# JeffOwOSun/ntm-tracker

Hardware: AMD Instinct MI355X
Metric: frames/sec (whole node) VGG16+NTM(128x20) seq_len=20 (higher is better)
Workload: dtype f32

## Files before the change

ntm-tracker_amd/csrc/conv_bf16p.hip:

```cpp
#include "conv_tiles.h"
#include "conv_stem.h"

#ifndef BF16P_ABL
#define BF16P_ABL 0
#endif

namespace {

typedef __bf16 pbf16x8 __attribute__((ext_vector_type(8)));
typedef __bf16 pbf16x4 __attribute__((ext_vector_type(4)));


struct Bf16pArgs {
    const __bf16* in; const __bf16* wq; const float* bias; void* out;
    int frames, H, W, Cin, Cout;
    int bxN, byN;
    int NQ, NS;
    int nCB;
    const float* stem_in = nullptr; const float* stem_w = nullptr; const float* stem_b = nullptr;
};

typedef int pv4i __attribute__((ext_vector_type(4)));
__device__ __forceinline__ void p_dma16(pv4i rs, unsigned lds_addr, int voff, int soff) {
    unsigned keep;
    asm volatile("s_mov_b32 %0, m0\n\ts_mov_b32 m0, %1\n\ts_nop 0\n\tbuffer_load_dwordx4 %2, %3, %4 offen lds\n\ts_mov_b32 m0, %0"
                 : "=&s"(keep) : "s"(lds_addr), "v"(voff), "s"(rs), "s"(soff) : "memory");
}
__device__ __forceinline__ pv4i p_rsrc(const void* base, unsigned bytes) {
    const unsigned long long p = (unsigned long long)base;
    return pv4i{(int)(unsigned)p, (int)(unsigned)(p >> 32), (int)bytes, 0x00020000};
}

__device__ __forceinline__ pbf16x8 p_as_bf16x8(const f32x4& v) {
    union { f32x4 f; pbf16x8 b; } u;
    u.f = v;
    return u.b;
}

typedef _Float16 ph16x8 __attribute__((ext_vector_type(8)));
typedef _Float16 ph16x4 __attribute__((ext_vector_type(4)));
typedef _Float16 ph16x2 __attribute__((ext_vector_type(2)));
__device__ __forceinline__ ph16x8 p_as_f16x8(const f32x4& v) {
    union { f32x4 f; ph16x8 h; } u;
    u.f = v;
    return u.h;
}
__device__ __forceinline__ void s3_split4(const f32x4& v, ph16x4& hi, ph16x4& lo) {
    const auto h01 = __builtin_amdgcn_cvt_pkrtz(v[0], v[1]), h23 = __builtin_amdgcn_cvt_pkrtz(v[2], v[3]);
    hi = ph16x4{(_Float16)h01[0], (_Float16)h01[1], (_Float16)h23[0], (_Float16)h23[1]};
#pragma unroll
    for (int e = 0; e < 4; ++e) lo[e] = (_Float16)(v[e] - (float)hi[e]);
}
constexpr float S3_MAX = 131008.f;

template <int PIECES>
__device__ __forceinline__ int p_sw(int idx) { return PIECES == 4 ? ((idx >> 2) & 3) : ((idx >> 3) & 1); }

template <int BN, int KC>
__global__ void bf16p_pack_kernel(const float* __restrict__ w, __bf16* __restrict__ wq, int Cin, int Cout) {
    constexpr int PIECES = KC / 8;
    const size_t total = (size_t)9 * Cin * Cout;
    const int NC = Cin / KC;
    for (size_t idx = (size_t)blockIdx.x * blockDim.x + threadIdx.x; idx < total; idx += (size_t)gridDim.x * blockDim.x) {
        const int e = idx & 7;
        size_t r = idx >> 3;
        const int slot = (int)(r % PIECES); r /= PIECES;
        const int n = (int)(r % BN); r /= BN;
        const int tap = (int)(r % 9); r /= 9;
        const int chunk = (int)(r % NC);
        const int cb = (int)(r / NC);
        const int piece = slot ^ p_sw<PIECES>(n);
        const int c = chunk * KC + piece * 8 + e;
        wq[idx] = (__bf16)w[((size_t)tap * Cin + c) * Cout + (size_t)cb * BN + n];
    }
}

__global__ void split3_absmax_kernel(const float* __restrict__ w, size_t n, unsigned* __restrict__ tail) {
    float m = 0.f;
    for (size_t i = (size_t)blockIdx.x * blockDim.x + threadIdx.x; i < n; i += (size_t)gridDim.x * blockDim.x) {
        const float v = fabsf(w[i]);
        if (v < 3.0e38f) m = fmaxf(m, v);
    }
#pragma unroll
    for (int o = 32; o > 0; o >>= 1) m = fmaxf(m, __shfl_xor(m, o));
    if ((threadIdx.x & 63) == 0) atomicMax(tail + 1, __float_as_uint(m));
}
__global__ void split3_scale_kernel(unsigned* __restrict__ tail) {
    const float m = __uint_as_float(tail[1]);
    int e = 0;
    if (m > 0.f) frexpf(m, &e);
    int k = 14 - e;
    k = k > 100 ? 100 : (k < -100 ? -100 : k);
    reinterpret_cast<float*>(tail)[0] = ldexpf(1.f, -k);
    reinterpret_cast<float*>(tail)[2] = ldexpf(1.f, k);
}
template <int BN>
__global__ void split3_pack_kernel(const float* __restrict__ w, _Float16* __restrict__ wq, int Cin, int Cout) {
    const size_t total = (size_t)18 * Cin * Cout;
    const float wscale = reinterpret_cast<const float*>(wq + total)[2];
    const int NC = Cin / 16;
    for (size_t idx = (size_t)blockIdx.x * blockDim.x + threadIdx.x; idx < total; idx += (size_t)gridDim.x * blockDim.x) {
        const int e = idx & 7;
        size_t r = idx >> 3;
        const int slot = (int)(r & 3); r >>= 2;
        const int n = (int)(r % BN); r /= BN;
        const int tap = (int)(r % 9); r /= 9;
        const int chunk = (int)(r % NC);
        const int cb = (int)(r / NC);
        const int piece = slot ^ p_sw<4>(n);
        const int c = chunk * 16 + (piece & 1) * 8 + e;
        const float v = w[((size_t)tap * Cin + c) * Cout + (size_t)cb * BN + n] * wscale;
        const _Float16 hi = (_Float16)v;
        wq[idx] = (piece & 2) ? (_Float16)(v - (float)hi) : hi;
    }
}

template <int BN, int TW, int TH, int NSUB, int KC, bool POOL, bool OUTF32, int NW = 8, bool X3 = false, bool INF32 = false, bool STEM = false>
__global__ __launch_bounds__(64 * NW) __attribute__((amdgpu_waves_per_eu(2, 2))) void conv3x3_relu_bf16p_kernel(Bf16pArgs a) {
    static_assert(!INF32 || (X3 && NW == 4), "fp32 input: split form on four waves (the eight-wave form has no registers for the staging)");
    static_assert(!STEM || (X3 && NW == 4 && !INF32 && (TW & (TW - 1)) == 0 && TW % 2 == 0), "fused stem: split form on four waves, sub-blocks");
    constexpr int PNT = 2 * NW;
    constexpr bool ROWS = (TW & (TW - 1)) != 0;
    static_assert(!X3 || KC == 32, "split form: 16 real channels = one 32-channel chunk");
    static_assert(!ROWS || (!POOL && NSUB == 1 && (TW - 1 + 32 * PNT - 1) / TW + 1 <= TH - 1 && NW == 8), "runs of rows: no row pairs; TH = the patch's image rows");
    static_assert(NW == 8 || (NW == 4 && BN == 64), "four-wave workgroups take 64 columns");
    constexpr int PW = ROWS ? 32 : TW + 2, PH = TH + 2, SPX = PW * PH, NPX = NSUB * SPX;
    static_assert(!ROWS || TW + 2 <= 32, "runs of rows: the patch row pitch is 32");
    constexpr int PIXB = KC * 2, PIECES = KC / 8, PPP = 1024 / PIXB;
    constexpr int NPA = (NPX + PPP - 1) / PPP;
    constexpr int ABYTES = STEM ? NPX * PIXB : NPA * 1024;
    constexpr int STAPS = KC == 16 ? 9 : 3, SPC = 9 / STAPS;
    constexpr int SBYTES = STAPS * BN * PIXB, NPB = SBYTES / 1024;
    constexpr int NPAW = (NPA + NW - 1) / NW;
    constexpr int TM = BN == 128 ? 4 : 2;
    constexpr int TPS = (TW * TH) / 32;
    constexpr int K16 = KC / 16;
    static_assert(ROWS || NSUB * TW * TH == 32 * PNT, "512 (256) output pixels per workgroup");
    constexpr int TRB = POOL ? 0 : NW * TM * 32 * 144;
    constexpr int LDSB = (2 * ABYTES + 2 * SBYTES) > TRB ? (2 * ABYTES + 2 * SBYTES) : TRB;
    constexpr int FPW = TW + 4, FPN = STEM ? NSUB * (TH + 4) * FPW * 3 : 4;
    constexpr int STEMB = STEM ? (FPN + 4 * 27 * 16 + 64) * 4 : 0;
    static_assert(LDSB + STEMB + 1024 <= ((NW == 8 || (STEM && NSUB > 1)) ? 160 : 80) * 1024, "LDS");
    __shared__ __attribute__((aligned(16))) float s_fp[FPN];
    __shared__ __attribute__((aligned(16))) float s_w1[STEM ? 4 * 27 * 16 : 4];
    __shared__ __attribute__((aligned(16))) float s_b1[STEM ? 64 : 4];
    __shared__ __attribute__((aligned(1024))) unsigned char s_mem[LDSB];
    __shared__ int s_sbf[NSUB], s_sby[NSUB], s_sbx[NSUB];
    __shared__ __attribute__((aligned(16))) float s_bias[BN + 4];

    const int tid = threadIdx.x, lane = tid & 63;
    const int wave = __builtin_amdgcn_readfirstlane(tid >> 6);
    int cb, sp;
    conv_tile_wg(blockIdx.x, a.nCB, cb, sp);
    if (sp >= a.NS) return;
    const int H = a.H, W = a.W, Cin = a.Cin, Cout = a.Cout;
    const int rP0 = sp * (32 * PNT), rg0 = ROWS ? rP0 / TW : 0, rf0 = ROWS ? rg0 / H : 0, ry0 = ROWS ? rg0 - rf0 * H : 0;
    if (tid < BN) s_bias[tid] = a.bias[cb * BN + tid];
    if (X3 && tid == BN) s_bias[BN] = *reinterpret_cast<const float*>(a.wq + (size_t)9 * a.Cin * a.Cout);
    if constexpr (!ROWS) conv_tile_subblocks<NSUB>(s_sbf, s_sby, s_sbx, tid, sp, a.NQ, a.bxN, a.byN, TH, TW, 0, 0);
    if constexpr (STEM) {
        for (int e = tid; e < 4 * 27 * 16; e += 64 * NW) {
            const int k = (e >> 4) % 27;
            s_w1[e] = a.stem_w[((e / (27 * 16)) * 16 + (e & 15)) * 32 + k];
        }
        if (tid < 64) s_b1[tid] = a.stem_b[tid];
    }
    __syncthreads();
    if constexpr (STEM) {
        for (int e = tid; e < FPN; e += 64 * NW) {
            int q, fy, fx, c, y, x;
            stem_fp_elem(e, TW, TH, q, fy, fx, c);
            const bool in = stem_fp_src(fy, fx, s_sby[q], s_sbx[q], H, W, y, x) && s_sbf[q] >= 0;
            s_fp[e] = in ? a.stem_in[(((size_t)s_sbf[q] * H + y) * W + x) * 3 + c] : 0.f;
        }
        __syncthreads();
    }

    auto a_sw = [](int p) { return ROWS ? ((((p & 31) + 28 * (p >> 5)) >> 2) & 3) : p_sw<PIECES>(p); };
    const int f0 = ROWS ? rf0 : ((sp * NSUB) / a.bxN) / a.byN;
    const size_t in_left = (size_t)(a.frames - f0) * H * W * Cin * sizeof(__bf16);
    const unsigned in_bytes = (unsigned)(in_left < 0x7ffffff0ull ? in_left : 0x7ffffff0ull);
    const __bf16* pin = a.in + (size_t)f0 * H * W * Cin;
    unsigned aoff[NPAW];
#pragma unroll
    for (int i = 0; i < NPAW; ++i) {
        const int pa = wave + NW * i;
        const int lp = pa * PPP + lane / PIECES, slot = lane % PIECES;
        aoff[i] = 0x80000000u;
        if (pa < NPA && lp < NPX) {
            const int q = lp / SPX, rem = lp - q * SPX;
            const int py = rem / PW, px = rem - py * PW;
            int fq, y;
            const int x = (ROWS ? 0 : s_sbx[q]) - 1 + px;
            if constexpr (ROWS) {
                const int U = ry0 + py, df = U / (H + 1);
                fq = rf0 + df; y = U - df * (H + 1) - 1;
                if (fq >= a.frames) fq = -1;
            } else {
                fq = s_sbf[q]; y = s_sby[q] - 1 + py;
            }
            if (fq >= 0 && y >= 0 && y < H && x >= 0 && x < W)
                aoff[i] = (unsigned)(((((size_t)(fq - f0) * H + y) * W + x) * Cin + (slot ^ a_sw(lp)) * 8) * sizeof(__bf16));
        }
    }
    constexpr int NIT = INF32 ? (NPX * 4 + 64 * NW - 1) / (64 * NW) : 1;
    constexpr int NITS = (NIT + SPC - 1) / SPC;
    unsigned foff[NIT];
    int fdst[NIT];
    if constexpr (INF32) {
#pragma unroll
        for (int i = 0; i < NIT; ++i) {
            const int it = tid + 64 * NW * i, lp = it >> 2, qd = it & 3;
            foff[i] = 0x80000000u; fdst[i] = -1;
            if (lp < NPX) {
                fdst[i] = lp * PIXB + (((qd >> 1) ^ a_sw(lp)) << 4) + (qd & 1) * 8;
                const int q = lp / SPX, rem = lp - q * SPX;
                const int py = rem / PW, px = rem - py * PW;
                const int fq = s_sbf[q];
                const int y = s_sby[q] - 1 + py, x = s_sbx[q] - 1 + px;
                if (fq >= 0 && y >= 0 && y < H && x >= 0 && x < W)
                    foff[i] = (unsigned)(((((size_t)(fq - f0) * H + y) * W + x) * Cin) * sizeof(__bf16) + qd * 16);
            }
        }
    }
    auto f32_rsrc = [&](int chunk) {
        return __builtin_amdgcn_make_buffer_rsrc(const_cast<__bf16*>(pin + (size_t)chunk * KC), 0, (int)(in_bytes - (unsigned)chunk * PIXB), 0x00020000);
    };
    auto f32_put = [&](const f32x4& v, int dst) {
        ph16x4 h, l;
        f32x4 c;
#pragma unroll
        for (int e = 0; e < 4; ++e) c[e] = __builtin_amdgcn_fmed3f(v[e], -S3_MAX, S3_MAX);
        s3_split4(c, h, l);
        *reinterpret_cast<ph16x4*>(s_mem + dst) = h;
        *reinterpret_cast<ph16x4*>(s_mem + (dst ^ 32)) = l;
    };
    constexpr int STILES = (NPX + 15) / 16;
    constexpr int SNIT = STEM ? (STILES + NW - 1) / NW : 1, SNITS = (SNIT + SPC - 1) / SPC;
    const int spi = lane & 15, sg = lane >> 4;
    int sfo[SNIT], skof[7];
    if constexpr (STEM) {
#pragma unroll
        for (int i = 0; i < SNIT; ++i) {
            const int lp = 16 * (wave + NW * i) + spi;
            sfo[i] = -1;
            if (lp < NPX) {
                int q, py, px;
                stem_pixel(lp, TW, TH, q, py, px);
                const bool in = s_sbf[q] >= 0 && stem_inside(py, px, s_sby[q], s_sbx[q], H, W);
                sfo[i] = stem_fp_corner(q, py, px, TW, TH) | (in ? 0 : 0x40000000);
            }
        }
#pragma unroll
        for (int s = 0; s < 7; ++s) skof[s] = 4 * s + sg < 27 ? stem_fp_k(4 * s + sg, TW) : 0;
    }
    float swa[7], sxs[SNITS][7];
    f32x4 sbv, sacc[SNITS];
    auto stem_load = [&](int chunk, int i, int j) {
        if (j == 0) {
#pragma unroll
            for (int s = 0; s < 7; ++s) swa[s] = 4 * s + sg < 27 ? s_w1[(chunk * 27 + 4 * s + sg) * 16 + spi] : 0.f;
            sbv = *reinterpret_cast<const f32x4*>(s_b1 + chunk * 16 + 4 * sg);
        }
        const float* fp = s_fp + (sfo[i] < 0 ? 0 : (sfo[i] & 0xffffff));
#pragma unroll
        for (int s = 0; s < 7; ++s) sxs[j][s] = 4 * s + sg < 27 ? fp[skof[s]] : 0.f;
    };
    auto stem_mfma = [&](int j, int s) {
        if (s == 0) sacc[j] = f32x4{0.f, 0.f, 0.f, 0.f};
        sacc[j] = __builtin_amdgcn_mfma_f32_16x16x4f32(swa[s], sxs[j][s], sacc[j], 0, 0, 0);
    };
    auto stem_put = [&](int i, int j, int buf) {
        if (sfo[i] < 0) return;
        const int lp = 16 * (wave + NW * i) + spi;
        const bool in = !(sfo[i] & 0x40000000);
        f32x4 v;
#pragma unroll
        for (int e = 0; e < 4; ++e) v[e] = in ? __builtin_amdgcn_fmed3f(sacc[j][e] + sbv[e], 0.f, S3_MAX) : 0.f;
        ph16x4 h, l;
        s3_split4(v, h, l);
        const int dst = buf * ABYTES + lp * PIXB + (((sg >> 1) ^ a_sw(lp)) << 4) + (sg & 1) * 8;
        *reinterpret_cast<ph16x4*>(s_mem + dst) = h;
        *reinterpret_cast<ph16x4*>(s_mem + (dst ^ 32)) = l;
    };
    const unsigned lds0 = (unsigned)(size_t)(__attribute__((address_space(3))) void*)s_mem;
    auto dma_patch = [&](int chunk, int buf, int i0, int i1) {
        const pv4i rs = p_rsrc(pin + (size_t)chunk * KC, in_bytes - (unsigned)chunk * PIXB);
#pragma unroll
        for (int i = 0; i < NPAW; ++i) {
            if (i >= i0 && i < i1 && wave + NW * i < NPA)
                p_dma16(rs, lds0 + buf * ABYTES + (wave + NW * i) * 1024, (int)aoff[i], 0);
        }
    };
    auto dma_patch1 = [&](int chunk, int buf, auto ic) {
        constexpr int i = decltype(ic)::value;
        const pv4i rs = p_rsrc(pin + (size_t)chunk * KC, in_bytes - (unsigned)chunk * PIXB);
        if (wave + NW * i < NPA) p_dma16(rs, lds0 + buf * ABYTES + (wave + NW * i) * 1024, (int)aoff[i], 0);
    };
    const int NC = Cin / KC, NSTG = SPC * NC;
    const pv4i wrs = p_rsrc(a.wq + (size_t)cb * NSTG * (SBYTES / 2), (unsigned)NSTG * SBYTES);
    auto dma_weights1 = [&](int stage, int buf, int i) {
        const int pb = wave + NW * i;
        if (pb < NPB) p_dma16(wrs, lds0 + 2 * ABYTES + buf * SBYTES + pb * 1024, lane * 16, stage * SBYTES + pb * 1024);
    };
    auto dma_weights = [&](int stage, int buf) {
#pragma unroll
        for (int i = 0; i < (NPB + NW - 1) / NW; ++i) {
            const int pb = wave + NW * i;
            if (pb < NPB) p_dma16(wrs, lds0 + 2 * ABYTES + buf * SBYTES + pb * 1024, lane * 16, stage * SBYTES + pb * 1024);
        }
    };

    const int wm = BN == 128 ? (wave >> 1) : wave, wn = BN == 128 ? (wave & 1) : 0;
    const int mcol = lane & 31, kh = lane >> 5;
    int pix0[TM];
    int opix[TM];
    auto locate = [&](int t, int m, int& pc, int& op) {
        if constexpr (ROWS) {
            const int P = rP0 + t * 32 + m;
            const int g = P / TW, x = P - g * TW, f = g / H, y = g - f * H;
            const bool real = f < a.frames;
            pc = real ? ((f - rf0) * (H + 1) + y + 1 - ry0) * PW + x + 1 : PW + 1;
            op = real ? P : -1;
        } else {
            int q, y, x;
            if constexpr (TPS == 0) {
                q = 2 * t + (m >> 4); y = (m >> 2) & 3; x = m & 3;
            } else {
                constexpr int RPT = 32 / TW;
                const int tl = t % TPS, j = m / TW;
                q = t / TPS;
                y = 2 * ((tl >> 1) * RPT + j) + (tl & 1);
                x = m % TW;
                if constexpr (TW == 16) x = (x + 12 * j) & 15;
                if constexpr (TW == 8) x ^= ((0x9 >> j) & 1) << 2;
            }
            pc = q * SPX + (y + 1) * PW + (x + 1);
            const int fq = s_sbf[q];
            const int Y = s_sby[q] + y, X = s_sbx[q] + x;
            if constexpr (POOL) op = fq < 0 ? -1 : ((fq * (H >> 1) + (Y >> 1)) * (W >> 1) + (X >> 1));
            else op = fq < 0 ? -1 : ((fq * H + Y) * W + X);
        }
    };
#pragma unroll
    for (int tm = 0; tm < TM; ++tm) locate(wm * TM + tm, mcol, pix0[tm], opix[tm]);
    int xa[9][TM];
#pragma unroll
    for (int tap = 0; tap < 9; ++tap)
#pragma unroll
        for (int tm = 0; tm < TM; ++tm) {
            const int p = pix0[tm] + (tap / 3 - 1) * PW + (tap % 3 - 1);
            xa[tap][tm] = p * PIXB + ((kh ^ a_sw(p)) << 4);
        }
    f32x16 acc[TM][2];
#pragma unroll
    for (int tm = 0; tm < TM; ++tm)
#pragma unroll
        for (int nt = 0; nt < 2; ++nt)
#pragma unroll
            for (int r = 0; r < 16; ++r) acc[tm][nt][r] = 0.f;
    const int wa0 = 2 * ABYTES + (wn * 64 + mcol) * PIXB + ((kh ^ p_sw<PIECES>(mcol)) << 4);

    if constexpr (INF32) {
        const __amdgpu_buffer_rsrc_t rs = f32_rsrc(0);
        f32x4 v[NIT];
#pragma unroll
        for (int i = 0; i < NIT; ++i) v[i] = __builtin_bit_cast(f32x4, __builtin_amdgcn_raw_buffer_load_b128(rs, (int)foff[i], 0, 0));
#pragma unroll
        for (int i = 0; i < NIT; ++i)
            if (fdst[i] >= 0) f32_put(v[i], fdst[i]);
    } else if constexpr (!STEM) {
        dma_patch(0, 0, 0, NPAW);
    }
    dma_weights(0, 0);
    if constexpr (STEM) {
#pragma unroll
        for (int i = 0; i < SNIT; ++i) {
            stem_load(0, i, 0);
#pragma unroll
            for (int s = 0; s < 7; ++s) stem_mfma(0, s);
            stem_put(i, 0, 0);
        }
    }
    asm volatile("s_waitcnt vmcnt(0)" ::: "memory");
    __syncthreads();

    auto stage_body = [&](int chunk, auto part_c) {
        constexpr int part = decltype(part_c)::value;
        const int s = SPC * chunk + part;
        const int abuf = chunk & 1, bbuf = s & 1;
        constexpr int NDW = (NPB + NW - 1) / NW;
        constexpr int NDP = (INF32 || STEM) ? 0 : (NPAW + SPC - 1) / SPC;
        const bool more_w = !(BF16P_ABL & 1) && s + 1 < NSTG, more_p = !(BF16P_ABL & 1) && chunk + 1 < NC;
        auto dma_slot = [&](auto kc) {
            constexpr int k = decltype(kc)::value;
            if constexpr (k < NDW) { if (more_w) dma_weights1(s + 1, bbuf ^ 1, k); }
            else if constexpr (k < NDW + NDP && part * NDP + (k - NDW) < NPAW) {
                if (more_p) dma_patch1(chunk + 1, abuf ^ 1, ntk_ic<part * NDP + (k - NDW)>{});
            }
        };
        constexpr int SPER = (7 * SNITS + 8) / 9;
        auto stem_slot = [&](auto kc) {
            if constexpr (STEM) {
                constexpr int k = decltype(kc)::value;
                if (more_p) {
#pragma unroll
                    for (int u = k * SPER; u < (k + 1) * SPER && u < 7 * SNITS; ++u) {
                        if (part * SNITS + u / 7 >= SNIT) continue;
                        stem_mfma(u / 7, u % 7);
                        if (u % 7 == 6) stem_put(part * SNITS + u / 7, u / 7, abuf ^ 1);
                    }
                }
            }
        };
        if constexpr (STEM) {
            if (more_p) {
#pragma unroll
                for (int j = 0; j < SNITS; ++j)
                    if (part * SNITS + j < SNIT) stem_load(chunk + 1, part * SNITS + j, j);
            }
        }
        const int wa = wa0 + bbuf * SBYTES;
        f32x4 fst[NITS];
        if constexpr (INF32) {
            const __amdgpu_buffer_rsrc_t rs = f32_rsrc(more_p ? chunk + 1 : chunk);
#pragma unroll
            for (int j = 0; j < NITS; ++j)
                if (part * NITS + j < NIT) fst[j] = __builtin_bit_cast(f32x4, __builtin_amdgcn_raw_buffer_load_b128(rs, (int)foff[part * NITS + j], 0, 0));
        }
        if constexpr (X3) {
            f32x4 wh[2][2], wl[2], xh[TM], xl[TM];
            auto ld_w = [&](auto dc, auto kc, f32x4 (&w)[2]) {
                constexpr int dxi = decltype(dc)::value, k16 = decltype(kc)::value;
#pragma unroll
                for (int nt = 0; nt < 2; ++nt)
                    w[nt] = *reinterpret_cast<const f32x4*>(s_mem + ((wa ^ (k16 << 5)) + (dxi * BN + nt * 32) * PIXB));
            };
            auto ld_x = [&](auto dc, auto kc, f32x4 (&x)[TM]) {
                constexpr int tap = part * STAPS + decltype(dc)::value, k16 = decltype(kc)::value;
#pragma unroll
                for (int tm = 0; tm < TM; ++tm) x[tm] = *reinterpret_cast<const f32x4*>(s_mem + (xa[tap][tm] ^ (k16 << 5)));
            };
            auto mm = [&](const f32x4 (&w)[2], const f32x4 (&x)[TM]) {
                if constexpr ((BF16P_ABL & 8) != 0) return;
#pragma unroll
                for (int tm = 0; tm < TM; ++tm)
#pragma unroll
                    for (int nt = 0; nt < 2; ++nt)
                        acc[tm][nt] = __builtin_amdgcn_mfma_f32_32x32x16_f16(p_as_f16x8(w[nt]), p_as_f16x8(x[tm]), acc[tm][nt], 0, 0, 0);
            };
            using I0 = ntk_ic<0>;
            using I1 = ntk_ic<1>;
            constexpr int NSS = STAPS * 3;
            static_assert(NDW + NDP <= NSS, "one DMA per sub-step");
            auto tapstep = [&](auto dc) {
                constexpr int dxi = decltype(dc)::value;
                if constexpr (!(BF16P_ABL & 4)) ld_w(dc, I1{}, wl);
                __builtin_amdgcn_sched_barrier(0);
                mm(wh[dxi & 1], xh);
                dma_slot(ntk_ic<3 * dxi>{});
                stem_slot(ntk_ic<3 * dxi>{});
                __builtin_amdgcn_sched_barrier(0);
                if constexpr (!(BF16P_ABL & 4)) ld_x(dc, I1{}, xl);
                __builtin_amdgcn_sched_barrier(0);
                mm(wl, xh);
                dma_slot(ntk_ic<3 * dxi + 1>{});
                stem_slot(ntk_ic<3 * dxi + 1>{});
                __builtin_amdgcn_sched_barrier(0);
                if constexpr (dxi + 1 < STAPS && !(BF16P_ABL & 4)) {
                    ld_w(ntk_ic<dxi + 1>{}, I0{}, wh[(dxi + 1) & 1]);
                    ld_x(ntk_ic<dxi + 1>{}, I0{}, xh);
                }
                __builtin_amdgcn_sched_barrier(0);
                mm(wh[dxi & 1], xl);
                dma_slot(ntk_ic<3 * dxi + 2>{});
                stem_slot(ntk_ic<3 * dxi + 2>{});
                __builtin_amdgcn_sched_barrier(0);
            };
            ld_w(I0{}, I0{}, wh[0]);
            ld_x(I0{}, I0{}, xh);
            if constexpr ((BF16P_ABL & 4) != 0) {
#pragma unroll
                for (int nt = 0; nt < 2; ++nt) { wh[1][nt] = wh[0][nt]; wl[nt] = wh[0][nt]; }
#pragma unroll
                for (int tm = 0; tm < TM; ++tm) xl[tm] = xh[tm];
            }
            ntk_static_for<0, STAPS>(tapstep);
            if constexpr (INF32) {
                if (more_p) {
#pragma unroll
                    for (int j = 0; j < NITS; ++j)
                        if (part * NITS + j < NIT && fdst[part * NITS + j] >= 0) f32_put(fst[j], (abuf ^ 1) * ABYTES + fdst[part * NITS + j]);
                }
            }
            if (!(BF16P_ABL & 2)) {
                asm volatile("s_waitcnt vmcnt(0)" ::: "memory");
                __syncthreads();
            }
            return;
        }
        constexpr int NSTEP = STAPS * K16;
        f32x4 wf[2][2], xf[2][TM];
        auto load_frags = [&](auto stc, f32x4 (&wfs)[2], f32x4 (&xfs)[TM]) {
            constexpr int st = decltype(stc)::value, dxi = st / K16, k16 = st % K16;
            constexpr int tap = part * STAPS + dxi;
#pragma unroll
            for (int nt = 0; nt < 2; ++nt)
                wfs[nt] = *reinterpret_cast<const f32x4*>(s_mem + ((wa ^ (k16 << 5)) + (dxi * BN + nt * 32) * PIXB));
#pragma unroll
            for (int tm = 0; tm < TM; ++tm) xfs[tm] = *reinterpret_cast<const f32x4*>(s_mem + (xa[tap][tm] ^ (k16 << 5)));
        };
        auto step = [&](auto stc) {
            constexpr int st = decltype(stc)::value;
            if constexpr (st + 1 < NSTEP && !(BF16P_ABL & 4)) load_frags(ntk_ic<st + 1>{}, wf[(st + 1) & 1], xf[(st + 1) & 1]);
            __builtin_amdgcn_sched_barrier(0);
            if constexpr ((BF16P_ABL & 8) != 0) return;
#pragma unroll
            for (int tm = 0; tm < TM; ++tm)
#pragma unroll
                for (int nt = 0; nt < 2; ++nt)
                    acc[tm][nt] = __builtin_amdgcn_mfma_f32_32x32x16_bf16(p_as_bf16x8(wf[(BF16P_ABL & 4) ? 0 : (st & 1)][nt]),
                                                                          p_as_bf16x8(xf[(BF16P_ABL & 4) ? 0 : (st & 1)][tm]), acc[tm][nt], 0, 0, 0);
            constexpr int PER = (NDW + NDP + NSTEP - 1) / NSTEP;
            dma_slot(ntk_ic<st * PER>{});
            if constexpr (PER > 1) dma_slot(ntk_ic<st * PER + 1>{});
            static_assert(PER <= 2, "DMAs per step");
            __builtin_amdgcn_sched_barrier(0);
        };
        if (!(BF16P_ABL & 4) || s == 0) load_frags(ntk_ic<0>{}, wf[0], xf[0]);
        ntk_static_for<0, NSTEP>(step);
        if (!(BF16P_ABL & 2)) {
            asm volatile("s_waitcnt vmcnt(0)" ::: "memory");
            __syncthreads();
        }
    };
    for (int chunk = 0; chunk < NC; ++chunk) {
        stage_body(chunk, ntk_ic<0>{});
        if constexpr (SPC > 1) {
            stage_body(chunk, ntk_ic<1>{});
            stage_body(chunk, ntk_ic<2>{});
        }
        const int flip = (chunk & 1) ? -ABYTES : ABYTES;
#pragma unroll
        for (int tap = 0; tap < 9; ++tap)
#pragma unroll
            for (int tm = 0; tm < TM; ++tm) xa[tap][tm] += flip;
    }

    if constexpr ((BF16P_ABL & 16) != 0) {
        float sacc = 0.f;
#pragma unroll
        for (int tm = 0; tm < TM; ++tm)
#pragma unroll
            for (int nt = 0; nt < 2; ++nt)
#pragma unroll
                for (int r = 0; r < 16; ++r) sacc += acc[tm][nt][r];
        if (sacc == 12345.f) reinterpret_cast<float*>(a.out)[tid] = sacc;
        return;
    }
    const int nbase = cb * BN + wn * 64 + 4 * kh;
    const float oscale = X3 ? s_bias[BN] : 1.f;
    if constexpr (POOL) {
#pragma unroll
        for (int nt = 0; nt < 2; ++nt)
#pragma unroll
            for (int g = 0; g < 4; ++g) {
                const int n = nbase + nt * 32 + 8 * g;
                const f32x4 bv = *reinterpret_cast<const f32x4*>(s_bias + n - cb * BN);
#pragma unroll
                for (int tm = 0; tm < TM; tm += 2) {
                    f32x4 v;
#pragma unroll
                    for (int e = 0; e < 4; ++e) {
                        const float m2 = fmaxf(acc[tm][nt][4 * g + e], acc[tm + 1][nt][4 * g + e]);
                        const float m4 = fmaxf(m2, ntk_dpp<0xB1>(m2));
                        if constexpr (X3 && !OUTF32) v[e] = __builtin_amdgcn_fmed3f(m4 * oscale + bv[e], 0.f, S3_MAX);
                        else v[e] = fmaxf((X3 ? m4 * oscale : m4) + bv[e], 0.f);
                    }
                    if (opix[tm] >= 0 && (mcol & 1) == 0) {
                        if constexpr (OUTF32) *reinterpret_cast<f32x4*>(reinterpret_cast<float*>(a.out) + (size_t)opix[tm] * Cout + n) = v;
                        else if constexpr (X3) {
                            ph16x4 oh, ol;
                            s3_split4(v, oh, ol);
                            _Float16* op = reinterpret_cast<_Float16*>(a.out) + (size_t)opix[tm] * (2 * Cout) + (n >> 4) * 32 + (n & 15);
                            *reinterpret_cast<ph16x4*>(op) = oh;
                            *reinterpret_cast<ph16x4*>(op + 16) = ol;
                        } else {
                            pbf16x4 o;
#pragma unroll
                            for (int e = 0; e < 4; ++e) o[e] = (__bf16)v[e];
                            *reinterpret_cast<pbf16x4*>(reinterpret_cast<__bf16*>(a.out) + (size_t)opix[tm] * Cout + n) = o;
                        }
                    }
                }
            }
    } else {
        constexpr int RB = 144;
        constexpr int WREG = TM * 32 * RB;
        static_assert(NW * WREG <= LDSB, "the transpose image fits");
        unsigned char* tr = s_mem + wave * WREG;
        constexpr bool WIDE = OUTF32 || X3;
        constexpr int NPASS = WIDE ? 2 : 1;
#pragma unroll
        for (int ps = 0; ps < NPASS; ++ps) {
#pragma unroll
            for (int nt = 0; nt < 2; ++nt) {
                if (WIDE && nt != ps) continue;
#pragma unroll
                for (int g = 0; g < 4; ++g) {
                    const f32x4 bv = *reinterpret_cast<const f32x4*>(s_bias + nbase - cb * BN + nt * 32 + 8 * g);
#pragma unroll
                    for (int tm = 0; tm < TM; ++tm) {
                        f32x4 v;
#pragma unroll
                        for (int e = 0; e < 4; ++e) {
                            if constexpr (X3 && !OUTF32) v[e] = __builtin_amdgcn_fmed3f(acc[tm][nt][4 * g + e] * oscale + bv[e], 0.f, S3_MAX);
                            else v[e] = fmaxf((X3 ? acc[tm][nt][4 * g + e] * oscale : acc[tm][nt][4 * g + e]) + bv[e], 0.f);
                        }
                        unsigned char* row = tr + (tm * 32 + mcol) * RB;
                        if constexpr (OUTF32) *reinterpret_cast<f32x4*>(row + (8 * g + 4 * kh) * 4) = v;
                        else if constexpr (X3) {
                            ph16x4 oh, ol;
                            s3_split4(v, oh, ol);
                            unsigned char* pr = row + (g >> 1) * 64 + ((g & 1) * 8 + 4 * kh) * 2;
                            *reinterpret_cast<ph16x4*>(pr) = oh;
                            *reinterpret_cast<ph16x4*>(pr + 32) = ol;
                        } else {
                            pbf16x4 o;
#pragma unroll
                            for (int e = 0; e < 4; ++e) o[e] = (__bf16)v[e];
                            *reinterpret_cast<pbf16x4*>(row + (nt * 32 + 8 * g + 4 * kh) * 2) = o;
                        }
                    }
                }
            }
#pragma unroll
            for (int j = 0; j < TM * 4; ++j) {
                const int tmr = j >> 2, mr = 8 * (j & 3) + (lane >> 3), piece = lane & 7;
                const f32x4 v = *reinterpret_cast<const f32x4*>(tr + (tmr * 32 + mr) * RB + piece * 16);
                const int opx = __builtin_amdgcn_ds_bpermute(mr << 2, opix[tmr]);
                if ((BF16P_ABL & 32) ? (opx >= 0 && v[0] == 12345.f) : (opx >= 0)) {
                    const size_t op = (size_t)opx * Cout + cb * BN + wn * 64;
                    if constexpr (OUTF32) *reinterpret_cast<f32x4*>(reinterpret_cast<float*>(a.out) + op + ps * 32 + piece * 4) = v;
                    else if constexpr (X3) *reinterpret_cast<f32x4*>(reinterpret_cast<__bf16*>(a.out) + 2 * (op + ps * 32) + piece * 8) = v;
                    else *reinterpret_cast<f32x4*>(reinterpret_cast<__bf16*>(a.out) + op + piece * 8) = v;
                }
            }
        }
    }
}

template <int BN, int KC, int NW, bool X3 = false, bool INF32 = false, bool STEM = false>
int bf16p_launch(const Bf16pArgs& a0, int H, int W, int pool, int out_f32, hipStream_t st) {
    Bf16pArgs a = a0;
    if constexpr (X3 && !INF32) {
        if (W == 28) {
            if (pool || NW != 8 || H < 20) return NTK_ERR_UNSUPPORTED;
            a.bxN = 1; a.byN = 1;
            const long long NQ = (long long)a.frames * H * W, NS = (NQ + 511) / 512;
            a.NQ = 0; a.NS = (int)NS; a.nCB = a.Cout / BN;
            const unsigned grid = (unsigned)conv_tile_grid(NS, a.nCB);
            if constexpr (NW == 8) {
                if (out_f32) conv3x3_relu_bf16p_kernel<BN, 28, 21, 1, 32, false, true, 8, true><<<grid, 512, 0, st>>>(a);
                else conv3x3_relu_bf16p_kernel<BN, 28, 21, 1, 32, false, false, 8, true><<<grid, 512, 0, st>>>(a);
            }
            return NTK_OK;
        }
    }
    int shape;
    if (NW == 8) shape = (W % 32 == 0 && H % 16 == 0) ? 0 : ((W % 16 == 0 && H % 16 == 0) ? 1 : ((W % 8 == 0 && H % 8 == 0) ? 2 : 3));
    else shape = (W % 32 == 0 && H % 8 == 0) ? 0 : ((W % 16 == 0 && H % 16 == 0) ? 1 : ((W % 8 == 0 && H % 8 == 0) ? 2 : 3));
    static const int TWs[4] = {32, 16, 8, 4}, THs8[4] = {16, 16, 8, 4}, THs4[4] = {8, 16, 8, 4}, NSUB8[4] = {1, 2, 8, 32}, NSUB4[4] = {1, 1, 4, 16};
    const int TWv = TWs[shape], THv = NW == 8 ? THs8[shape] : THs4[shape], NSUBv = NW == 8 ? NSUB8[shape] : NSUB4[shape];
    a.bxN = W / TWv;
    a.byN = H / THv;
    const long long NQ = (long long)a.frames * a.bxN * a.byN;
    const long long NS = (NQ + NSUBv - 1) / NSUBv;
    a.NQ = (int)NQ; a.NS = (int)NS; a.nCB = a.Cout / BN;
    const unsigned grid = (unsigned)conv_tile_grid(NS, a.nCB);
#define BF16P_GO(TW_, TH_, NSUB_)                                                                                             \
    do {                                                                                                                      \
        if (pool) {                                                                                                           \
            if (out_f32) conv3x3_relu_bf16p_kernel<BN, TW_, TH_, NSUB_, KC, true, true, NW, X3, INF32, STEM><<<grid, 64 * NW, 0, st>>>(a);     \
            else conv3x3_relu_bf16p_kernel<BN, TW_, TH_, NSUB_, KC, true, false, NW, X3, INF32, STEM><<<grid, 64 * NW, 0, st>>>(a);            \
        } else {                                                                                                              \
            if (out_f32) conv3x3_relu_bf16p_kernel<BN, TW_, TH_, NSUB_, KC, false, true, NW, X3, INF32, STEM><<<grid, 64 * NW, 0, st>>>(a);    \
            else conv3x3_relu_bf16p_kernel<BN, TW_, TH_, NSUB_, KC, false, false, NW, X3, INF32, STEM><<<grid, 64 * NW, 0, st>>>(a);           \
        }                                                                                                                     \
    } while (0)
    if constexpr (KC == 32 && NW == 8) {
        if (shape == 0) BF16P_GO(32, 16, 1);
        else if (shape == 1) BF16P_GO(16, 16, 2);
        else if (shape == 2) BF16P_GO(8, 8, 8);
        else return NTK_ERR_UNSUPPORTED;
    } else if constexpr (KC == 32) {
        if (shape == 0) BF16P_GO(32, 8, 1);
        else if (shape == 1) BF16P_GO(16, 16, 1);
        else if (shape == 2) BF16P_GO(8, 8, 4);
        else return NTK_ERR_UNSUPPORTED;
    } else {
        if (shape == 3 && !pool && NW == 8) {
            if (out_f32) conv3x3_relu_bf16p_kernel<BN, 4, 4, 32, KC, false, true><<<grid, 512, 0, st>>>(a);
            else conv3x3_relu_bf16p_kernel<BN, 4, 4, 32, KC, false, false><<<grid, 512, 0, st>>>(a);
        } else return NTK_ERR_UNSUPPORTED;
    }
#undef BF16P_GO
    return NTK_OK;
}

}

static int bf16p_form(int H, int W, int cin, int cout, int pool, int* bn, int* kc, int* nw) {
    if (H <= 0 || W <= 0 || cin <= 0 || cout <= 0 || (H % 4) || (W % 4) || cin % 32 || cout % 64) return 0;
    const bool rect = (W % 8 == 0 && H % 8 == 0);
    if (!rect && pool) return 0;
    *nw = (rect && cin <= 64 && cout == 64) ? 4 : 8;
    *bn = (*nw == 8 && cout % 128 == 0) ? 128 : 64;
    *kc = rect ? 32 : 16;
    return conv_tile_ncb_ok(cout / *bn);
}

extern "C" size_t ntk_vgg_bf16p_packed_elems(int cin, int cout) { return (size_t)9 * cin * cout; }

extern "C" int ntk_vgg_pack_weights_bf16p(const float* w_hwio, void* w_packed_bf16, int cin, int cout, int H, int W, void* stream) {
    NTK_REQUIRE(w_hwio && w_packed_bf16, NTK_ERR_BAD_PTR, "ntk_vgg_pack_weights_bf16p: null pointer");
    int bn = 0, kc = 0, nw = 0;
    NTK_REQUIRE(bf16p_form(H, W, cin, cout, 0, &bn, &kc, &nw), NTK_ERR_UNSUPPORTED,
                "ntk_vgg_pack_weights_bf16p: cin=%d (multiple of 32) cout=%d (multiple of 64) H=%d W=%d (multiples of 4)", cin, cout, H, W);
    __bf16* wq = reinterpret_cast<__bf16*>(w_packed_bf16);
    hipStream_t st = (hipStream_t)stream;
    if (bn == 128 && kc == 32) bf16p_pack_kernel<128, 32><<<1024, 256, 0, st>>>(w_hwio, wq, cin, cout);
    else if (bn == 64 && kc == 32) bf16p_pack_kernel<64, 32><<<1024, 256, 0, st>>>(w_hwio, wq, cin, cout);
    else if (bn == 128) bf16p_pack_kernel<128, 16><<<1024, 256, 0, st>>>(w_hwio, wq, cin, cout);
    else bf16p_pack_kernel<64, 16><<<1024, 256, 0, st>>>(w_hwio, wq, cin, cout);
    NTK_CHECK_LAUNCH("ntk_vgg_pack_weights_bf16p");
    return NTK_OK;
}

extern "C" int ntk_vgg_bf16p_supported(int H, int W, int cin, int cout, int fuse_pool) {
    int bn = 0, kc = 0, nw = 0;
    return bf16p_form(H, W, cin, cout, fuse_pool, &bn, &kc, &nw);
}

extern "C" int ntk_vgg_conv3x3_relu_bf16p(const void* in_bf16, const void* w_packed_bf16p, const float* bias, void* out,
                                          int frames, int H, int W, int cin, int cout, int fuse_pool, int out_f32, void* stream) {
    NTK_REQUIRE(in_bf16 && w_packed_bf16p && bias && out, NTK_ERR_BAD_PTR, "ntk_vgg_conv3x3_relu_bf16p: null pointer");
    NTK_REQUIRE(ntk_aligned16(in_bf16) && ntk_aligned16(w_packed_bf16p) && ntk_aligned16(out) && ntk_aligned16(bias), NTK_ERR_BAD_PTR,
                "ntk_vgg_conv3x3_relu_bf16p: pointers must be 16-byte aligned");
    int bn = 0, kc = 0, nw = 0;
    NTK_REQUIRE(frames > 0 && H > 0 && W > 0 && bf16p_form(H, W, cin, cout, fuse_pool, &bn, &kc, &nw), NTK_ERR_UNSUPPORTED,
                "ntk_vgg_conv3x3_relu_bf16p: frames=%d H=%d W=%d cin=%d cout=%d pool=%d (H, W multiples of 4 -- of 8 with the pool; "
                "cin a multiple of 32, cout of 64)", frames, H, W, cin, cout, fuse_pool);
    NTK_REQUIRE((unsigned long long)2 * H * W * cin * sizeof(__bf16) <= 0x7ffffff0ull && (long long)frames * H * W < (1ll << 31), NTK_ERR_UNSUPPORTED,
                "ntk_vgg_conv3x3_relu_bf16p: frame too large for 32-bit offsets");
    Bf16pArgs a;
    a.in = reinterpret_cast<const __bf16*>(in_bf16); a.wq = reinterpret_cast<const __bf16*>(w_packed_bf16p); a.bias = bias; a.out = out;
    a.frames = frames; a.H = H; a.W = W; a.Cin = cin; a.Cout = cout;
    a.bxN = a.byN = a.NQ = a.NS = a.nCB = 0;
    int rc;
    hipStream_t st = (hipStream_t)stream;
    if (nw == 4) rc = bf16p_launch<64, 32, 4>(a, H, W, fuse_pool, out_f32, st);
    else if (bn == 128 && kc == 32) rc = bf16p_launch<128, 32, 8>(a, H, W, fuse_pool, out_f32, st);
    else if (bn == 64 && kc == 32) rc = bf16p_launch<64, 32, 8>(a, H, W, fuse_pool, out_f32, st);
    else if (bn == 128) rc = bf16p_launch<128, 16, 8>(a, H, W, fuse_pool, out_f32, st);
    else rc = bf16p_launch<64, 16, 8>(a, H, W, fuse_pool, out_f32, st);
    NTK_REQUIRE(rc == NTK_OK, rc, "ntk_vgg_conv3x3_relu_bf16p: no instantiation for this shape");
    NTK_CHECK_LAUNCH("ntk_vgg_conv3x3_relu_bf16p");
    return NTK_OK;
}


static int split3_form(int H, int W, int cin, int cout, int pool, int* bn, int* nw) {
    if (H <= 0 || W <= 0 || cin <= 0 || cout <= 0 || cin % 16 || cout % 64) return 0;
    const bool rect = (W % 8 == 0 && H % 8 == 0);
    if (!rect && (pool || W != 28 || H < 20)) return 0;
    *nw = (rect && cin <= 64 && cout == 64) ? 4 : 8;
    *bn = (*nw == 8 && cout % 128 == 0) ? 128 : 64;
    return conv_tile_ncb_ok(cout / *bn);
}

extern "C" size_t ntk_vgg_split3_packed_elems(int cin, int cout) { return (size_t)18 * cin * cout + 8; }

extern "C" int ntk_vgg_split3_supported(int H, int W, int cin, int cout, int fuse_pool) {
    int bn = 0, nw = 0;
    return split3_form(H, W, cin, cout, fuse_pool, &bn, &nw);
}

extern "C" int ntk_vgg_pack_weights_split3(const float* w_hwio, void* w_packed, int cin, int cout, int H, int W, void* stream) {
    NTK_REQUIRE(w_hwio && w_packed, NTK_ERR_BAD_PTR, "ntk_vgg_pack_weights_split3: null pointer");
    int bn = 0, nw = 0;
    NTK_REQUIRE(split3_form(H, W, cin, cout, 0, &bn, &nw), NTK_ERR_UNSUPPORTED,
                "ntk_vgg_pack_weights_split3: cin=%d (multiple of 16) cout=%d (multiple of 64) H=%d W=%d", cin, cout, H, W);
    _Float16* wq = reinterpret_cast<_Float16*>(w_packed);
    hipStream_t st = (hipStream_t)stream;
    unsigned* tail = reinterpret_cast<unsigned*>(wq + (size_t)18 * cin * cout);
    if (hipMemsetAsync(tail, 0, 16, st) != hipSuccess) return NTK_ERR_HIP;
    split3_absmax_kernel<<<256, 256, 0, st>>>(w_hwio, (size_t)9 * cin * cout, tail);
    split3_scale_kernel<<<1, 1, 0, st>>>(tail);
    if (bn == 128) split3_pack_kernel<128><<<1024, 256, 0, st>>>(w_hwio, wq, cin, cout);
    else split3_pack_kernel<64><<<1024, 256, 0, st>>>(w_hwio, wq, cin, cout);
    NTK_CHECK_LAUNCH("ntk_vgg_pack_weights_split3");
    return NTK_OK;
}

extern "C" int ntk_vgg_conv3x3_relu_split3(const void* in_split, const void* w_packed, const float* bias, void* out,
                                           int frames, int H, int W, int cin, int cout, int fuse_pool, int in_f32, int out_f32, void* stream) {
    NTK_REQUIRE(in_split && w_packed && bias && out, NTK_ERR_BAD_PTR, "ntk_vgg_conv3x3_relu_split3: null pointer");
    NTK_REQUIRE(ntk_aligned16(in_split) && ntk_aligned16(w_packed) && ntk_aligned16(out) && ntk_aligned16(bias), NTK_ERR_BAD_PTR,
                "ntk_vgg_conv3x3_relu_split3: pointers must be 16-byte aligned");
    int bn = 0, nw = 0;
    NTK_REQUIRE(frames > 0 && H > 0 && W > 0 && split3_form(H, W, cin, cout, fuse_pool, &bn, &nw), NTK_ERR_UNSUPPORTED,
                "ntk_vgg_conv3x3_relu_split3: frames=%d H=%d W=%d cin=%d cout=%d pool=%d (H, W multiples of 8, or W = 28 and H >= 20 "
                "without the pool; cin a multiple of 16, cout of 64)", frames, H, W, cin, cout, fuse_pool);
    NTK_REQUIRE((unsigned long long)2 * H * W * cin * 4 <= 0x7ffffff0ull && (long long)frames * H * W < (1ll << 31), NTK_ERR_UNSUPPORTED,
                "ntk_vgg_conv3x3_relu_split3: frame too large for 32-bit offsets");
    Bf16pArgs a;
    a.in = reinterpret_cast<const __bf16*>(in_split); a.wq = reinterpret_cast<const __bf16*>(w_packed); a.bias = bias; a.out = out;
    a.frames = frames; a.H = H; a.W = W; a.Cin = 2 * cin; a.Cout = cout;
    a.bxN = a.byN = a.NQ = a.NS = a.nCB = 0;
    int rc;
    hipStream_t st = (hipStream_t)stream;
    NTK_REQUIRE(!in_f32 || nw == 4, NTK_ERR_UNSUPPORTED,
                "ntk_vgg_conv3x3_relu_split3: an fp32 input map is read by the four-wave form only (cin <= 64, cout = 64, H and W multiples of 8)");
    if (nw == 4 && in_f32) rc = bf16p_launch<64, 32, 4, true, true>(a, H, W, fuse_pool, out_f32, st);
    else if (nw == 4) rc = bf16p_launch<64, 32, 4, true>(a, H, W, fuse_pool, out_f32, st);
    else if (bn == 128) rc = bf16p_launch<128, 32, 8, true>(a, H, W, fuse_pool, out_f32, st);
    else rc = bf16p_launch<64, 32, 8, true>(a, H, W, fuse_pool, out_f32, st);
    NTK_REQUIRE(rc == NTK_OK, rc, "ntk_vgg_conv3x3_relu_split3: no instantiation for this shape");
    NTK_CHECK_LAUNCH("ntk_vgg_conv3x3_relu_split3");
    return NTK_OK;
}

extern "C" int ntk_vgg_split3_stem_supported(int H, int W, int fuse_pool) {
    int bn = 0, nw = 0;
    return split3_form(H, W, 64, 64, fuse_pool, &bn, &nw) && nw == 4 && (W % 8) == 0 && (H % 8) == 0;
}

extern "C" int ntk_vgg_conv3x3_relu_split3_stem(const float* frames_f32, const float* w1_packed, const float* bias1, const void* w2_packed,
                                                const float* bias2, void* out, int frames, int H, int W, int fuse_pool, int out_f32,
                                                void* stream) {
    NTK_REQUIRE(frames_f32 && w1_packed && bias1 && w2_packed && bias2 && out, NTK_ERR_BAD_PTR, "ntk_vgg_conv3x3_relu_split3_stem: null pointer");
    NTK_REQUIRE(ntk_aligned16(w2_packed) && ntk_aligned16(out) && ntk_aligned16(bias2) && (((uintptr_t)frames_f32 | (uintptr_t)w1_packed | (uintptr_t)bias1) & 3u) == 0,
                NTK_ERR_BAD_PTR, "ntk_vgg_conv3x3_relu_split3_stem: w2_packed, bias2 and out must be 16-byte aligned, the rest 4-byte");
    NTK_REQUIRE(frames > 0 && H > 0 && W > 0 && ntk_vgg_split3_stem_supported(H, W, fuse_pool), NTK_ERR_UNSUPPORTED,
                "ntk_vgg_conv3x3_relu_split3_stem: frames=%d H=%d W=%d pool=%d (H, W multiples of 8)", frames, H, W, fuse_pool);
    NTK_REQUIRE((long long)frames * H * W < (1ll << 31), NTK_ERR_UNSUPPORTED, "ntk_vgg_conv3x3_relu_split3_stem: too many pixels for 32-bit offsets");
    Bf16pArgs a;
    a.in = nullptr; a.wq = reinterpret_cast<const __bf16*>(w2_packed); a.bias = bias2; a.out = out;
    a.frames = frames; a.H = H; a.W = W; a.Cin = 128; a.Cout = 64;
    a.bxN = a.byN = a.NQ = a.NS = a.nCB = 0;
    a.stem_in = frames_f32; a.stem_w = w1_packed; a.stem_b = bias1;
    const int rc = bf16p_launch<64, 32, 4, true, false, true>(a, H, W, fuse_pool, out_f32, (hipStream_t)stream);
    NTK_REQUIRE(rc == NTK_OK, rc, "ntk_vgg_conv3x3_relu_split3_stem: no instantiation for this shape");
    NTK_CHECK_LAUNCH("ntk_vgg_conv3x3_relu_split3_stem");
    return NTK_OK;
}
```

Baseline: 14320.

## Pipeline X3 conv epilogue stores and use fused fp16 split and lane swaps

Rewrites the X3 (split-fp16) epilogue of the bf16p conv kernel. The non-pool path now processes the output in four quarter-chunks, overlapping LDS transpose fetches and global stores of one chunk with the compute of the next. A wave-uniform fast path drops the per-row bounds checks when all output pixels are inside. A faster hi/lo split uses v_fma_mix_f32, scale and bias are applied with a vector fma, and in the pool path permlane32_swap merges hi and lo halves so each lane issues one 16-byte store instead of two 8-byte stores. These changes target epilogue instruction count and store latency, at the cost of higher register pressure and use of inline asm that is specific to this architecture.

New measurement: 14300. About the same (-0.1%).

```diff
diff --git a/ntm-tracker_amd/csrc/conv_bf16p.hip b/ntm-tracker_amd/csrc/conv_bf16p.hip
--- a/ntm-tracker_amd/csrc/conv_bf16p.hip
+++ b/ntm-tracker_amd/csrc/conv_bf16p.hip
@@ -40,6 +40,8 @@
 typedef _Float16 ph16x8 __attribute__((ext_vector_type(8)));
 typedef _Float16 ph16x4 __attribute__((ext_vector_type(4)));
 typedef _Float16 ph16x2 __attribute__((ext_vector_type(2)));
+typedef unsigned u32x2 __attribute__((ext_vector_type(2)));
+typedef unsigned u32x4 __attribute__((ext_vector_type(4)));
 __device__ __forceinline__ ph16x8 p_as_f16x8(const f32x4& v) {
     union { f32x4 f; ph16x8 h; } u;
     u.f = v;
@@ -52,6 +54,21 @@
     for (int e = 0; e < 4; ++e) lo[e] = (_Float16)(v[e] - (float)hi[e]);
 }
 constexpr float S3_MAX = 131008.f;
+__device__ __forceinline__ void s3_split4_fast(const f32x4& v, ph16x4& hi, ph16x4& lo) {
+    const ph16x2 h01 = __builtin_bit_cast(ph16x2, __builtin_amdgcn_cvt_pkrtz(v[0], v[1]));
+    const ph16x2 h23 = __builtin_bit_cast(ph16x2, __builtin_amdgcn_cvt_pkrtz(v[2], v[3]));
+    const unsigned u01 = __builtin_bit_cast(unsigned, h01), u23 = __builtin_bit_cast(unsigned, h23);
+    float d0, d1, d2, d3;
+    asm("v_fma_mix_f32 %0, %1, -1.0, %2 op_sel_hi:[1,0,0]" : "=v"(d0) : "v"(u01), "v"(v[0]));
+    asm("v_fma_mix_f32 %0, %1, -1.0, %2 op_sel:[1,0,0] op_sel_hi:[1,0,0]" : "=v"(d1) : "v"(u01), "v"(v[1]));
+    asm("v_fma_mix_f32 %0, %1, -1.0, %2 op_sel_hi:[1,0,0]" : "=v"(d2) : "v"(u23), "v"(v[2]));
+    asm("v_fma_mix_f32 %0, %1, -1.0, %2 op_sel:[1,0,0] op_sel_hi:[1,0,0]" : "=v"(d3) : "v"(u23), "v"(v[3]));
+    hi = ph16x4{h01[0], h01[1], h23[0], h23[1]};
+    lo = __builtin_convertvector(f32x4{d0, d1, d2, d3}, ph16x4);
+}
+__device__ __forceinline__ f32x4 s3_scale_bias4(const f32x4& acc, float scale, const f32x4& bias) {
+    return __builtin_elementwise_fma(acc, f32x4{scale, scale, scale, scale}, bias);
+}
 
 template <int PIECES>
 __device__ __forceinline__ int p_sw(int idx) { return PIECES == 4 ? ((idx >> 2) & 3) : ((idx >> 3) & 1); }
@@ -561,6 +578,12 @@
     const int nbase = cb * BN + wn * 64 + 4 * kh;
     const float oscale = X3 ? s_bias[BN] : 1.f;
     if constexpr (POOL) {
+        _Float16* sp16[TM / 2];
+        if constexpr (X3 && !OUTF32) {
+#pragma unroll
+            for (int tm = 0; tm < TM; tm += 2)
+                sp16[tm / 2] = reinterpret_cast<_Float16*>(a.out) + (size_t)opix[tm] * (2 * Cout) + ((cb * BN + wn * 64) >> 4) * 32 + 16 * kh;
+        }
 #pragma unroll
         for (int nt = 0; nt < 2; ++nt)
 #pragma unroll
@@ -573,19 +596,27 @@
 #pragma unroll
                     for (int e = 0; e < 4; ++e) {
                         const float m2 = fmaxf(acc[tm][nt][4 * g + e], acc[tm + 1][nt][4 * g + e]);
-                        const float m4 = fmaxf(m2, ntk_dpp<0xB1>(m2));
-                        if constexpr (X3 && !OUTF32) v[e] = __builtin_amdgcn_fmed3f(m4 * oscale + bv[e], 0.f, S3_MAX);
-                        else v[e] = fmaxf((X3 ? m4 * oscale : m4) + bv[e], 0.f);
+                        v[e] = fmaxf(m2, ntk_dpp<0xB1>(m2));
                     }
-                    if (opix[tm] >= 0 && (mcol & 1) == 0) {
+                    if constexpr (X3) {
+                        v = s3_scale_bias4(v, oscale, bv);
+#pragma unroll
+                        for (int e = 0; e < 4; ++e) v[e] = OUTF32 ? fmaxf(v[e], 0.f) : __builtin_amdgcn_fmed3f(v[e], 0.f, S3_MAX);
+                    } else {
+#pragma unroll
+                        for (int e = 0; e < 4; ++e) v[e] = fmaxf(v[e] + bv[e], 0.f);
+                    }
+                    const bool mine = opix[tm] >= 0 && (mcol & 1) == 0;
+                    if constexpr (X3 && !OUTF32) {
+                        ph16x4 oh, ol;
+                        s3_split4_fast(v, oh, ol);
+                        const u32x2 uh = __builtin_bit_cast(u32x2, oh), ul = __builtin_bit_cast(u32x2, ol);
+                        const auto r0 = __builtin_amdgcn_permlane32_swap(uh[0], ul[0], false, false);
+                        const auto r1 = __builtin_amdgcn_permlane32_swap(uh[1], ul[1], false, false);
+                        if (mine) *reinterpret_cast<u32x4*>(sp16[tm / 2] + (nt * 2 + (g >> 1)) * 32 + (g & 1) * 8) = u32x4{r0[0], r1[0], r0[1], r1[1]};
+                    } else if (mine) {
                         if constexpr (OUTF32) *reinterpret_cast<f32x4*>(reinterpret_cast<float*>(a.out) + (size_t)opix[tm] * Cout + n) = v;
-                        else if constexpr (X3) {
-                            ph16x4 oh, ol;
-                            s3_split4(v, oh, ol);
-                            _Float16* op = reinterpret_cast<_Float16*>(a.out) + (size_t)opix[tm] * (2 * Cout) + (n >> 4) * 32 + (n & 15);
-                            *reinterpret_cast<ph16x4*>(op) = oh;
-                            *reinterpret_cast<ph16x4*>(op + 16) = ol;
-                        } else {
+                        else {
                             pbf16x4 o;
 #pragma unroll
                             for (int e = 0; e < 4; ++e) o[e] = (__bf16)v[e];
@@ -599,51 +630,101 @@
         constexpr int WREG = TM * 32 * RB;
         static_assert(NW * WREG <= LDSB, "the transpose image fits");
         unsigned char* tr = s_mem + wave * WREG;
-        constexpr bool WIDE = OUTF32 || X3;
-        constexpr int NPASS = WIDE ? 2 : 1;
-#pragma unroll
-        for (int ps = 0; ps < NPASS; ++ps) {
-#pragma unroll
-            for (int nt = 0; nt < 2; ++nt) {
-                if (WIDE && nt != ps) continue;
+        if constexpr (X3) {
+            constexpr int HT = TM / 2, NPC = HT * 4;
+            auto compute = [&](auto kc) {
+                constexpr int k = decltype(kc)::value, nt = k >> 1, th = k & 1;
 #pragma unroll
                 for (int g = 0; g < 4; ++g) {
                     const f32x4 bv = *reinterpret_cast<const f32x4*>(s_bias + nbase - cb * BN + nt * 32 + 8 * g);
 #pragma unroll
-                    for (int tm = 0; tm < TM; ++tm) {
-                        f32x4 v;
-#pragma unroll
-                        for (int e = 0; e < 4; ++e) {
-                            if constexpr (X3 && !OUTF32) v[e] = __builtin_amdgcn_fmed3f(acc[tm][nt][4 * g + e] * oscale + bv[e], 0.f, S3_MAX);
-                            else v[e] = fmaxf((X3 ? acc[tm][nt][4 * g + e] * oscale : acc[tm][nt][4 * g + e]) + bv[e], 0.f);
-                        }
+                    for (int tm = th * HT; tm < (th + 1) * HT; ++tm) {
+                        f32x4 v = s3_scale_bias4(f32x4{acc[tm][nt][4 * g], acc[tm][nt][4 * g + 1], acc[tm][nt][4 * g + 2], acc[tm][nt][4 * g + 3]}, oscale, bv);
+#pragma unroll
+                        for (int e = 0; e < 4; ++e) v[e] = OUTF32 ? fmaxf(v[e], 0.f) : __builtin_amdgcn_fmed3f(v[e], 0.f, S3_MAX);
                         unsigned char* row = tr + (tm * 32 + mcol) * RB;
                         if constexpr (OUTF32) *reinterpret_cast<f32x4*>(row + (8 * g + 4 * kh) * 4) = v;
-                        else if constexpr (X3) {
+                        else {
                             ph16x4 oh, ol;
-                            s3_split4(v, oh, ol);
+                            s3_split4_fast(v, oh, ol);
                             unsigned char* pr = row + (g >> 1) * 64 + ((g & 1) * 8 + 4 * kh) * 2;
                             *reinterpret_cast<ph16x4*>(pr) = oh;
                             *reinterpret_cast<ph16x4*>(pr + 32) = ol;
-                        } else {
-                            pbf16x4 o;
-#pragma unroll
-                            for (int e = 0; e < 4; ++e) o[e] = (__bf16)v[e];
-                            *reinterpret_cast<pbf16x4*>(row + (nt * 32 + 8 * g + 4 * kh) * 2) = o;
                         }
                     }
                 }
-            }
-#pragma unroll
-            for (int j = 0; j < TM * 4; ++j) {
-                const int tmr = j >> 2, mr = 8 * (j & 3) + (lane >> 3), piece = lane & 7;
-                const f32x4 v = *reinterpret_cast<const f32x4*>(tr + (tmr * 32 + mr) * RB + piece * 16);
-                const int opx = __builtin_amdgcn_ds_bpermute(mr << 2, opix[tmr]);
-                if ((BF16P_ABL & 32) ? (opx >= 0 && v[0] == 12345.f) : (opx >= 0)) {
-                    const size_t op = (size_t)opx * Cout + cb * BN + wn * 64;
-                    if constexpr (OUTF32) *reinterpret_cast<f32x4*>(reinterpret_cast<float*>(a.out) + op + ps * 32 + piece * 4) = v;
-                    else if constexpr (X3) *reinterpret_cast<f32x4*>(reinterpret_cast<__bf16*>(a.out) + 2 * (op + ps * 32) + piece * 8) = v;
-                    else *reinterpret_cast<f32x4*>(reinterpret_cast<__bf16*>(a.out) + op + piece * 8) = v;
+            };
+            auto fetch = [&](auto kc, f32x4 (&rv)[NPC], int (&ox)[NPC]) {
+                constexpr int th = decltype(kc)::value & 1;
+#pragma unroll
+                for (int j = 0; j < NPC; ++j) {
+                    const int tmr = th * HT + (j >> 2), mr = 8 * (j & 3) + (lane >> 3), piece = lane & 7;
+                    rv[j] = *reinterpret_cast<const f32x4*>(tr + (tmr * 32 + mr) * RB + piece * 16);
+                    ox[j] = __builtin_amdgcn_ds_bpermute(mr << 2, opix[tmr]);
+                }
+            };
+            unsigned char* const ob = reinterpret_cast<unsigned char*>(a.out) + (size_t)(cb * BN + wn * 64) * 4 + (lane & 7) * 16;
+            auto put = [&](auto kc, auto allc, const f32x4 (&rv)[NPC], const int (&ox)[NPC]) {
+                constexpr int ps = decltype(kc)::value >> 1;
+                constexpr bool ALL = decltype(allc)::value;
+#pragma unroll
+                for (int j = 0; j < NPC; ++j) {
+                    if (((BF16P_ABL & 32) ? rv[j][0] == 12345.f : true) && (ALL || ox[j] >= 0))
+                        *reinterpret_cast<f32x4*>(ob + (size_t)ox[j] * Cout * 4 + ps * 128) = rv[j];
+                }
+            };
+            auto run = [&](auto allc) {
+                f32x4 rv[NPC];
+                int ox[NPC];
+                compute(ntk_ic<0>{});
+                ntk_static_for<0, 4>([&](auto kc) {
+                    constexpr int k = decltype(kc)::value;
+                    fetch(kc, rv, ox);
+                    if constexpr (k + 1 < 4) compute(ntk_ic<k + 1>{});
+                    put(kc, allc, rv, ox);
+                });
+            };
+            bool inside = true;
+#pragma unroll
+            for (int tm = 0; tm < TM; ++tm) inside = inside && opix[tm] >= 0;
+            if (__builtin_amdgcn_ballot_w64(!inside) == 0) run(ntk_ic<1>{});
+            else run(ntk_ic<0>{});
+        } else {
+            constexpr int NPASS = OUTF32 ? 2 : 1;
+#pragma unroll
+            for (int ps = 0; ps < NPASS; ++ps) {
+#pragma unroll
+                for (int nt = 0; nt < 2; ++nt) {
+                    if (OUTF32 && nt != ps) continue;
+#pragma unroll
+                    for (int g = 0; g < 4; ++g) {
+                        const f32x4 bv = *reinterpret_cast<const f32x4*>(s_bias + nbase - cb * BN + nt * 32 + 8 * g);
+#pragma unroll
+                        for (int tm = 0; tm < TM; ++tm) {
+                            f32x4 v;
+#pragma unroll
+                            for (int e = 0; e < 4; ++e) v[e] = fmaxf(acc[tm][nt][4 * g + e] + bv[e], 0.f);
+                            unsigned char* row = tr + (tm * 32 + mcol) * RB;
+                            if constexpr (OUTF32) *reinterpret_cast<f32x4*>(row + (8 * g + 4 * kh) * 4) = v;
+                            else {
+                                pbf16x4 o;
+#pragma unroll
+                                for (int e = 0; e < 4; ++e) o[e] = (__bf16)v[e];
+                                *reinterpret_cast<pbf16x4*>(row + (nt * 32 + 8 * g + 4 * kh) * 2) = o;
+                            }
+                        }
+                    }
+                }
+#pragma unroll
+                for (int j = 0; j < TM * 4; ++j) {
+                    const int tmr = j >> 2, mr = 8 * (j & 3) + (lane >> 3), piece = lane & 7;
+                    const f32x4 v = *reinterpret_cast<const f32x4*>(tr + (tmr * 32 + mr) * RB + piece * 16);
+                    const int opx = __builtin_amdgcn_ds_bpermute(mr << 2, opix[tmr]);
+                    if ((BF16P_ABL & 32) ? (opx >= 0 && v[0] == 12345.f) : (opx >= 0)) {
+                        const size_t op = (size_t)opx * Cout + cb * BN + wn * 64;
+                        if constexpr (OUTF32) *reinterpret_cast<f32x4*>(reinterpret_cast<float*>(a.out) + op + ps * 32 + piece * 4) = v;
+                        else *reinterpret_cast<f32x4*>(reinterpret_cast<__bf16*>(a.out) + op + piece * 8) = v;
+                    }
                 }
             }
         }
```
